# jzebedee/deltaq

Hardware: AMD Instinct MI355X
Metric: MB of text suffix-sorted per second (bit-exact SA) (higher is better)
Workload: dtype u8 text / u64 keys / int32 SA; 1 GPU; 256 MiB uniform-random bytes per GPU (splitmix64 seed 0x5EED0003+rank), int32 SA; bytes_per_gpu=268435456, residency=text and SA resident in HBM, rounds_after_initial_sort=1

## Files before the change

deltaq_amd/csrc/dq_bucket_sort.h:

```cpp
#pragma once
#include "dq_onesweep.h"
#include "dq_round0_plan.h"

namespace dq {

constexpr int kBktBins = kBktCap;
constexpr int kBktMaxBin = 48;

struct BucketFlags {
    unsigned long long overflow;
};

static __global__ __launch_bounds__(kBlock) void bucket_bounds_kernel(const uint64_t *__restrict__ W, int64_t n, int bshift,
                                                               int64_t C, int64_t X, int64_t ntiles,
                                                               int64_t *__restrict__ bounds,
                                                               BucketFlags *__restrict__ flags)
{
    const int64_t t = (int64_t)blockIdx.x * kBlock + threadIdx.x;
    if (t > ntiles) return;
    if (t == ntiles) { bounds[t] = n; return; }
    if (t == 0) { bounds[0] = 0; return; }
    const int64_t p = t * C;
    const uint64_t b = W[p - 1] >> bshift;
    int64_t lo = p, hi = p + X < n ? p + X : n;
// ... 17 lines not shown
    const int64_t b = (int64_t)blockIdx.x * kBlock + threadIdx.x;
    if (b > nbuckets) return;
    if (b == nbuckets) { bounds[ntiles] = n; return; }
    int64_t lo = 0, hi = n;
    while (lo < hi) {
        const int64_t mid = lo + ((hi - lo) >> 1);
        if ((int64_t)(W[mid] >> bshift) < b) lo = mid + 1; else hi = mid;
    }
    if (lo + X < n && (int64_t)(W[lo + X] >> bshift) == b) atomicOr(&flags->overflow, 2ull);
    if (b % g == 0) bounds[b / g] = lo;
}

template <int kThreads, int kItems, int kWavesPerSimd>
struct BktGeometry {
    static constexpr int threads = kThreads, items = kItems, waves = kWavesPerSimd;
    static constexpr int cap = kThreads * kItems;
    static constexpr int nb = 2 * cap;
    static_assert(cap < (1 << 16) && (nb / 2) % kThreads == 0 && kThreads % kWave == 0, "16-bit starts; whole bin words per thread");
};
using BktCoarse = BktGeometry<1024, kBktCap / 1024, 4>;
using BktFine = BktGeometry<512, kBktCapFine / 512, 4>;
static_assert(BktCoarse::cap == kBktCap && BktFine::cap == kBktCapFine, "the tiles are cut for these capacities");
constexpr int kBktArrBits = 6;
constexpr int kBktWalk = 4;
static_assert(kBktMaxBin < (1 << kBktArrBits), "arrival numbers must fit");

#ifdef DQ_BKT_PHASE_TIMING
__device__ long long *g_bkt_ts = nullptr;
#define DQ_BKT_PHASE(i) do { if (threadIdx.x == 0 && g_bkt_ts) g_bkt_ts[(long long)tile * 16 + (i)] = clock64(); } while (0)
#else
#define DQ_BKT_PHASE(i) do { } while (0)
#endif

template <typename IdxT, bool kExt = false, typename G = BktCoarse>
__global__ __launch_bounds__(G::threads, G::waves) void bucket_sort_kernel(
    const uint64_t *__restrict__ W, int ib, int lowbits, const int64_t *__restrict__ bounds, int64_t ntiles,
    IdxT *__restrict__ SA, uint32_t *__restrict__ ebits, BucketFlags *__restrict__ flags,
    const uint8_t *__restrict__ E = nullptr)
{
    constexpr int kCap = G::cap, kThreads = G::threads, kNB = G::nb, kItems = G::items;
    constexpr int kBinsPerThread = kNB / kThreads;
    constexpr int kWords = kBinsPerThread / 2;
    __shared__ uint32_t buf[kCap + kBktWalk];
    __shared__ uint32_t bins[kNB / 2 + 2];
    __shared__ uint32_t sufs[kCap];
    __shared__ uint32_t wtot[kThreads / kWave];
    __shared__ uint64_t s_edge[2];
    __shared__ uint32_t s_overflow;

    const uint32_t tid = threadIdx.x;
    const int lane = lane_id();
    const uint32_t wv = tid >> 6;
    const int bshift = ib + lowbits;
    const uint32_t imask = (uint32_t)((1ull << ib) - 1);
    const uint16_t *start16 = reinterpret_cast<const uint16_t *>(bins);

    int64_t tile = blockIdx.x;
    if (tile >= ntiles) return;
    int64_t lo_n = bounds[tile];
    uint32_t M_n = (uint32_t)(bounds[tile + 1] - lo_n);
    if (M_n > (uint32_t)kCap) M_n = 0;
    int64_t lo_nn = 0, hi_nn = 0;
    if (tile + gridDim.x < ntiles) { lo_nn = bounds[tile + gridDim.x]; hi_nn = bounds[tile + gridDim.x + 1]; }
    uint64_t wd[kItems];
#define DQ_BKT_FETCH()                                                            \
    do {                                                                          \
        const uint64_t *Wn = W + (M_n ? lo_n : 0);    \
        const uint32_t last_ = M_n > 0 ? M_n - 1 : 0;                             \
        _Pragma("unroll") for (int k = 0; k < kItems; ++k) {                   \
            const uint32_t e_ = (uint32_t)(k * kThreads) + tid;                \
            wd[k] = Wn[e_ < last_ ? e_ : last_];                                  \
        }                                                                         \
    } while (0)
#define DQ_BKT_REQUEST_NEXT()                                                     \
    do {                                                                          \
        lo_n = lo_nn;                                                             \
        M_n = (uint32_t)(hi_nn - lo_nn);                                          \
        if (M_n > (uint32_t)kCap) M_n = 0;                                     \
        DQ_BKT_FETCH();                                                           \
        if (tn + gridDim.x < ntiles) { lo_nn = bounds[tn + gridDim.x]; hi_nn = bounds[tn + gridDim.x + 1]; } \
    } while (0)
    DQ_BKT_FETCH();

    for (;;) {
        const int64_t lo = lo_n;
        const uint32_t M = M_n;
        const int64_t tn = tile + gridDim.x;
        if (M == 0) {
            if (tn >= ntiles) break;
            DQ_BKT_REQUEST_NEXT();
            tile = tn;
            continue;
        }
        DQ_BKT_PHASE(0);
        uint32_t ex[kExt ? kItems : 1];
        if (kExt) {
            const uint8_t *En = E + lo;
            const uint32_t last_ = M - 1;
#pragma unroll
            for (int k = 0; k < kItems; ++k) {
                const uint32_t e_ = (uint32_t)(k * kThreads) + tid;
                ex[k] = En[e_ < last_ ? e_ : last_];
            }
        }
        const int lowbits_t = kExt ? lowbits + 8 : lowbits;
        if (tid == 0) { s_edge[0] = wd[0]; s_overflow = 0; }
        if (tid == kThreads - 1) s_edge[1] = wd[kItems - 1];
        for (uint32_t i = tid; i < (uint32_t)(kNB / 2 + 2); i += kThreads) bins[i] = 0;
        __syncthreads();
        DQ_BKT_PHASE(1);
        const uint64_t kfirst = s_edge[0] >> bshift, klast = s_edge[1] >> bshift;
        const uint64_t range = (klast - kfirst + 1) << lowbits_t;
        const bool bad = range > (1ull << (32 - kBktArrBits));
        const uint32_t mult = bad ? 0u
            : (uint32_t)fminf((float)kNB * 4294967296.0f * __frcp_rn((float)range) * (1.0f - 0x1p-20f), 4294967040.0f);
        const uint64_t kbase = kfirst << lowbits;
        uint32_t key[kItems];
#pragma unroll
// ... 67 lines not shown
                        const uint32_t bin = __umulhi(key[k] >> kBktArrBits, mult);
                        const uint32_t s0 = start16[bin], s1 = start16[bin + 1];
                        r = s0;
                        if (s1 > s0 + 1) {
#pragma unroll
                        for (int q = 0; q < kBktWalk; ++q) {
                            const uint32_t o = buf[s0 + q];
                            const uint32_t less = (s0 + q < s1) & (o < key[k]);
                            r += less;
                            tie |= less & ((o >> kBktArrBits) == (key[k] >> kBktArrBits));
                        }
                        }
                        if (s1 > s0 + kBktWalk) {
#pragma clang loop vectorize(disable) interleave(disable) unroll(disable)
                            for (uint32_t j = s0 + kBktWalk; j < s1; ++j) {
                                const uint32_t o = buf[j];
                                const uint32_t less = o < key[k];
                                r += less;
                                tie |= less & ((o >> kBktArrBits) == (key[k] >> kBktArrBits));
                            }
                        }
                    }
                    fin[k] = e < M ? (r | (tie << 31)) : 0xffffffffu;
                }
                __syncthreads();
                DQ_BKT_PHASE(5);
#pragma unroll
                for (int k = 0; k < kItems; ++k) {
                    if (fin[k] != 0xffffffffu)
                        buf[fin[k] & 0x7fffffffu] = sufs[k * kThreads + tid] | (fin[k] & 0x80000000u);
                }
                __syncthreads();
                DQ_BKT_PHASE(6);
                IdxT *out = SA + lo;
                uint32_t v[kItems];
#pragma unroll
                for (int k = 0; k < kItems; ++k) {
                    const uint32_t e = (uint32_t)(k * kThreads) + tid;
                    v[k] = buf[e < M ? e : 0];
                }
                uint32_t ties = 0;
#pragma unroll
                for (int k = 0; k < kItems; ++k) {
                    const uint32_t e = (uint32_t)(k * kThreads) + tid;
                    if (e < M) out[e] = (IdxT)(v[k] & 0x7fffffffu);
                    ties |= (e < M && (v[k] >> 31)) ? (1u << k) : 0u;
                }
                while (ties) {
                    const int k = __builtin_ctz(ties);
                    ties &= ties - 1;
                    const uint64_t o = (uint64_t)(lo + k * kThreads + tid);
                    atomicOr(&ebits[o >> 5], 1u << ((uint32_t)o & 31u));
                }
                DQ_BKT_PHASE(7);
            }
        }
        if (tn >= ntiles) break;
        tile = tn;
        __syncthreads();
    }
#undef DQ_BKT_REQUEST_NEXT
#undef DQ_BKT_FETCH
}

}
```

deltaq_amd/csrc/dq_flags.h:

```cpp
#pragma once

#include <algorithm>
#include <cstdint>
#include <cstdlib>
#include <cstring>
#include <optional>
#include <string>

namespace dq {

struct Flags {
    bool debug = false;
    std::optional<int> trace;
    std::optional<int> hip_device;
    std::optional<int> numa_bind;
    std::optional<std::string> fault;
    std::optional<int> small_n;
    std::optional<int> no_many;
    std::optional<int> mid_many_min;
    std::optional<int> no_large_many;
    std::optional<int> large_many_min;
    std::optional<int> no_diff_many;
    std::optional<int> no_diff_mid_many;
    std::optional<int> diff_mid_many_min;
    std::optional<int> no_diff_large;
    std::optional<int> diff_large_min;
    std::optional<int> diff_large_table;
    std::optional<int> no_index_many;
    std::optional<int> index_many_min;
    std::optional<int> index_many_threads;
    std::optional<int> no_index_large;
    std::optional<int> index_large_min;
    std::optional<int> no_check_many;
    std::optional<int> no_bwt_many;
    std::optional<int> no_mtf_many;
    std::optional<int> no_huff_many;
    std::optional<int> mtf_short_max;
    bool no_list_buffers = false;
    bool text_copy = false;
    bool assume_doubled = false;
    bool no_twins = false;
    bool no_period_hint = false;
    std::optional<int> xcd_group;
    std::optional<int> packed;
    std::optional<int> key_bytes;
    std::optional<int> coded;
    std::optional<int> split;
    bool no_bucket = false;
    std::optional<int> bucket;
    std::optional<int> bucket_keybits;
    std::optional<int> bucket_ext;
    std::optional<int> bucket_tile;
    bool old_first_pass = false;
    bool no_fused_ties = false;
    std::optional<int> sparse;
    std::optional<int> binned_isa;
    bool no_binned_isa = false;
    std::optional<int> runs;
    bool no_small = false;
    bool no_wide_small = false;
    bool no_first_small = false;
    std::optional<int> mid_groups;
    bool no_l_shift = false;
    bool no_upd_words = false;
    std::optional<int> upd_bin;
    std::optional<int> upd_bin_min;
    std::optional<int> upd_window;
    std::optional<int> chain_steps;
    bool no_chain = false;
    bool force_rshift = false;
    std::optional<int> tail_max;
    std::optional<int> pair_chains;
    std::optional<int> pair_chains_min;
    std::optional<int> pair_maxg;
    std::optional<int> late_runs_min;
    bool no_late_runs = false;
    std::optional<int> run_period;
    bool search_wave = false;
    std::optional<int> search_ptab;
    bool no_wave_windows = false;
    bool no_poll = false;
    bool no_second_stage = false;
    std::optional<int> win_min;
    std::optional<int> win_second;
    std::optional<int> walk_on;
// ... 42 lines not shown
    f.large_many_min = num("DQ_LARGE_MANY_MIN", 1);
    f.no_diff_many = num("DQ_NO_DIFF_MANY", 0, 1);
    f.no_diff_mid_many = num("DQ_NO_DIFF_MID_MANY", 0, 1);
    f.diff_mid_many_min = num("DQ_DIFF_MID_MANY_MIN", 1);
    f.no_diff_large = num("DQ_NO_DIFF_LARGE", 0, 1);
    f.diff_large_min = num("DQ_DIFF_LARGE_MIN", 1);
    f.diff_large_table = num("DQ_DIFF_LARGE_TABLE", 0, 1);
    f.no_index_many = num("DQ_NO_INDEX_MANY", 0, 1);
    f.index_many_min = num("DQ_INDEX_MANY_MIN", 1);
    f.index_many_threads = num("DQ_INDEX_MANY_THREADS");
    f.no_index_large = num("DQ_NO_INDEX_LARGE", 0, 1);
    f.index_large_min = num("DQ_INDEX_LARGE_MIN", 1);
    f.no_check_many = num("DQ_NO_CHECK_MANY", 0, 1);
    f.no_bwt_many = num("DQ_NO_BWT_MANY", 0, 1);
    f.no_mtf_many = num("DQ_NO_MTF_MANY", 0, 1);
    f.no_huff_many = num("DQ_NO_HUFF_MANY", 0, 1);
    f.mtf_short_max = num("DQ_MTF_SHORT_MAX", 0);
    f.no_list_buffers = on("DQ_NO_LIST_BUFFERS");
    f.text_copy = on("DQ_TEXT_COPY");
    f.assume_doubled = on("DQ_ASSUME_DOUBLED");
    f.no_twins = on("DQ_NO_TWINS");
    f.no_period_hint = on("DQ_NO_PERIOD_HINT");

    f.xcd_group = num("DQ_XCD_GROUP", 0, 64);
    f.packed = num("DQ_PACKED");
    f.key_bytes = num("DQ_KEY_BYTES", 1, 8);
    f.coded = num("DQ_CODED");
    f.split = num("DQ_SPLIT");
    f.no_bucket = on("DQ_NO_BUCKET");
    f.bucket = num("DQ_BUCKET");
    f.bucket_keybits = num("DQ_BUCKET_KEYBITS");
    f.bucket_ext = num("DQ_BUCKET_EXT");
    f.bucket_tile = num("DQ_BUCKET_TILE", 0, 1);
    f.old_first_pass = on("DQ_OLD_FIRST_PASS");
    f.no_fused_ties = on("DQ_NO_FUSED_TIES");
    f.sparse = num("DQ_SPARSE");
    f.binned_isa = num("DQ_BINNED_ISA");
    f.no_binned_isa = on("DQ_NO_BINNED_ISA");
    f.runs = num("DQ_RUNS");

    f.no_small = on("DQ_NO_SMALL");
    f.no_wide_small = on("DQ_NO_WIDE_SMALL");
    f.no_first_small = on("DQ_NO_FIRST_SMALL");
    f.mid_groups = num("DQ_MID_GROUPS");
    f.no_l_shift = on("DQ_NO_L_SHIFT");
    f.no_upd_words = on("DQ_NO_UPD_WORDS");
    f.upd_bin = num("DQ_UPD_BIN", 0, 2);
    f.upd_bin_min = num("DQ_UPD_BIN_MIN", 1);
    f.upd_window = num("DQ_UPD_WINDOW");
    f.chain_steps = num("DQ_CHAIN_STEPS");
    f.no_chain = on("DQ_NO_CHAIN");
    f.force_rshift = on("DQ_FORCE_RSHIFT");

    f.tail_max = num("DQ_TAIL_MAX", 0);
    f.pair_chains = num("DQ_PAIR_CHAINS");
    f.pair_chains_min = num("DQ_PAIR_CHAINS_MIN", 1);
    f.pair_maxg = num("DQ_PAIR_MAXG", 2);
    f.late_runs_min = num("DQ_LATE_RUNS_MIN", 1);
    f.no_late_runs = on("DQ_NO_LATE_RUNS");
    f.run_period = num("DQ_RUN_PERIOD", 1);

    f.search_wave = on("DQ_SEARCH_WAVE");
    f.search_ptab = num("DQ_SEARCH_PTAB");
    f.no_wave_windows = on("DQ_NO_WAVE_WINDOWS");
    f.no_poll = on("DQ_NO_POLL");
    f.no_second_stage = on("DQ_NO_SECOND_STAGE");
// ... 78 lines not shown
```

deltaq_amd/csrc/dq_round0.h:

```cpp
#pragma once
#include "dq_sort_passes.h"
#include "dq_alpha_code.h"
#include "dq_ties.h"
#include "dq_bucket_sort.h"
#include "dq_xcd_rank.h"

namespace dq {
namespace {

constexpr int64_t kSgShortList = 1 << 20;
inline int mid_group_cap(int64_t list_len)
{
    if (const std::optional<int> g = flags().mid_groups) {
        return *g >= 1024 ? 1024 : *g >= 512 ? 512 : *g >= 256 ? 256 : 0;
    }
    return list_len >= kSgShortList ? 512 : 1024;
}
inline bool small_round_usable(int64_t n, int64_t mm, bool third_list_buffer)
{
    const Flags &F = flags();
    return !F.no_small && n < (1ll << 32) && (mm * 2 <= n || (third_list_buffer && !F.no_wide_small));
}

template <typename Fn>
int with_bool(bool on, Fn fn)
{
    return on ? fn(std::true_type{}) : fn(std::false_type{});
}

constexpr int kXcdHistAt = kRadixSize + 16;

template <typename IdxT>
struct Round0Out {
    uint64_t *Kr[2] = {nullptr, nullptr};
    IdxT *Vr[2] = {nullptr, nullptr};
    int64_t m = 0, h = 0;
    int rbits = 0;
    bool dense_built = false;
// ... 181 lines not shown
        DQ_TRY(isa_from_suffix_words<IdxT>(L, c, w, n, ib, k.kb, P0, keys));
        if (list_rank && o.m == 0) return DQ_OK;
        if (list_rank && small_round_usable(n, o.m, third) && rank32_direct) {
            o.first_rank32 = list_rank;
            return DQ_OK;
        }
        if (list_rank && small_round_usable(n, o.m, third)) {
            LAUNCH(L, DQ_K_KEY2_FROM_PAIRS, o.m, o.m * 12,
                   hipLaunchKernelGGL(widen_ranks_kernel, dim3(grid_for(o.m)), dim3(kBlock), 0, st,
                                      (const uint32_t *)list_rank, o.m, keys));
            return DQ_OK;
        }
        const bool with_key2 = !o.runs.runs_wanted;
        const int kbits = bit_length((uint64_t)(n - 1) + (uint64_t)k.kb);
        unsigned long long *cnt = reinterpret_cast<unsigned long long *>(w.totals + 3);
        HIP_TRY(hipMemsetAsync(cnt, 0, 8, st));
        const int64_t per = (int64_t)kPairThreads * kPairItems;
        LAUNCH(L, DQ_K_KEY2_FROM_PAIRS, n, n * 8 + o.m * (wb + 8 + wb),
               hipLaunchKernelGGL(key2_from_pairs_kernel<IdxT>, dim3((unsigned)((n + per - 1) / per)), dim3(kPairThreads),
                                  0, st, (const uint64_t *)P0, n, ib, (const IdxT *)w.ISA, (int64_t)k.kb, kbits, with_key2,
                                  keys, w.Va, cnt));
        o.keys_ready = with_key2;
        o.list_ungrouped = true;
        return DQ_OK;
    }

    int bucketed(bool *done)
    {
        *done = false;
        const Flags &F = flags();
        const BucketPlan b = plan_bucketed(s, F, k, coded, (int)wb);
        if (!b.applies) return DQ_OK;
        const int kb = k.kb, keybits = b.keybits, lowbits = b.lowbits;
        uint8_t *E[2] = {reinterpret_cast<uint8_t *>(w.Va), reinterpret_cast<uint8_t *>(w.Va) + align_up((size_t)n)};
        uint32_t *ebits = reinterpret_cast<uint32_t *>(w.Vb);
        TieCounters *ctr = reinterpret_cast<TieCounters *>(w.totals + 6);
        BucketFlags *bflags = reinterpret_cast<BucketFlags *>(&ctr->overflow);
        hipLaunchKernelGGL(text_digit_offsets_kernel, dim3(b.bbytes), dim3(kBlock), 0, st,
                           (const int64_t *)w.bytehist, (const uint8_t *)w.text, n, b.bbytes, w.digit_offset,
                           b.xcd_pass ? (const int64_t *)(w.bytehist + kXcdHistAt) : nullptr, b.xcd_pass ? w.xcd_offset : nullptr);
        HIP_TRY(hipGetLastError());
        if (c.ncu <= 0) {
            int v = 0;
            c.ncu = hipDeviceGetAttribute(&v, hipDeviceAttributeMultiprocessorCount, c.dev) == hipSuccess && v > 0 ? v : 256;
        }
        if (b.xcd_pass) {
            if (F.trace) fprintf(stderr, "[dq] XCD-local first pass (n=%lld, eighths of %lld)\n", (long long)n, (long long)xcd_eighth(n));
            if (sizeof(XcdRankCtl) > w.ctl_status_stride) return fail(DQ_ERR_HIP, "status buffer too small");
            LAUNCH(L, DQ_K_RADIX_RANK, n, n * (1 + 8),
                   hipLaunchKernelGGL(xcd_text_rank_kernel, dim3((unsigned)std::min<int64_t>(c.ncu, (n + kXcdTileN - 1) / kXcdTileN)),
                                      dim3(kXcdRankThreads), 0, st, reinterpret_cast<const uint32_t *>(w.text), K[1], n,
                                      ib + lowbits, keybits, ib, (const int64_t *)w.xcd_offset,
                                      reinterpret_cast<XcdRankCtl *>(w.ctl_status)));
        } else {
            DQ_TRY(b.ext ? rank_pass_ext<IdxT, kTextPackedExt>(L, w, text64(), (const uint8_t *)nullptr, K[1], E[1], n, 0, ib, ib + lowbits, keybits)
                       : rank_pass<IdxT, kTextPacked>(L, w, text64(), (const IdxT *)nullptr, K[1], (IdxT *)nullptr, n, 0, kb, ib,
                                                      nullptr, nullptr, ib + lowbits, keybits));
        }
        for (int p = 1; p < b.bbytes; ++p) {
            DQ_TRY(b.ext ? rank_pass_ext<IdxT, kKeysExt>(L, w, K[p & 1], E[p & 1], K[(p & 1) ^ 1], E[(p & 1) ^ 1], n, p, ib, ib + lowbits + 8 * p, keybits)
                       : rank_pass<IdxT, kKeys>(L, w, K[p & 1], (const IdxT *)nullptr, K[(p & 1) ^ 1], (IdxT *)nullptr, n, p, kb, ib,
                                                nullptr, nullptr, ib + lowbits + 8 * p, keybits));
        }
        uint64_t *Ks = K[b.bbytes & 1], *Kfree = K[(b.bbytes & 1) ^ 1];
        const uint8_t *Es = b.ext ? E[b.bbytes & 1] : nullptr;
        const FinishTiles ft = plan_finish_tiles(b, n, F);
        if (F.trace)
            fprintf(stderr, "[dq] bucket finish: %s geometry, %lld tiles of up to %lld words cut every %lld %s (n=%lld)\n", ft.fine ? "fine" : "coarse",
                    (long long)ft.ntiles, (long long)ft.cap, (long long)(ft.by_id ? ft.g : ft.Cf), ft.by_id ? "buckets" : "words", (long long)n);
        if ((size_t)ft.ntiles + 1 > finish_bounds_entries(n)) return fail(DQ_ERR_HIP, "tile bounds buffer too small");
        if (ft.by_id) {
            const int64_t nbuckets = (int64_t)1 << (8 * b.bbytes);
            LAUNCH(L, DQ_K_BUCKET_SORT, ft.ntiles, ft.ntiles * 16 * 8,
                   hipLaunchKernelGGL(bucket_bounds_by_id_kernel, dim3((unsigned)((nbuckets + 1 + kBlock - 1) / kBlock)), dim3(kBlock), 0,
                                      st, (const uint64_t *)Ks, n, ib + lowbits, ft.g, b.X, nbuckets, ft.ntiles, w.bkt_bounds, bflags));
        } else {
            LAUNCH(L, DQ_K_BUCKET_SORT, ft.ntiles, ft.ntiles * 16 * 8,
                   hipLaunchKernelGGL(bucket_bounds_kernel, dim3((unsigned)((ft.ntiles + 1 + kBlock - 1) / kBlock)), dim3(kBlock), 0,
                                      st, (const uint64_t *)Ks, n, ib + lowbits, ft.Cf, b.X, ft.ntiles, w.bkt_bounds, bflags));
        }
        auto finish = [&](auto kExt, auto geometry) -> int {
            using G = decltype(geometry);
            auto kernel = bucket_sort_kernel<IdxT, decltype(kExt)::value, G>;
            const int groups = resident_groups(&c.bkt_groups[ft.fine][b.ext][sizeof(IdxT) == 8], (const void *)kernel, G::threads, c.dev);
            LAUNCH(L, DQ_K_BUCKET_SORT, n, n * ((b.ext ? 9 : 8) + wb) + n / 8,
                   hipLaunchKernelGGL(kernel, dim3((unsigned)std::min<int64_t>(ft.ntiles, groups)), dim3(G::threads), 0, st,
                                      (const uint64_t *)Ks, ib, lowbits, (const int64_t *)w.bkt_bounds, ft.ntiles, d_sa, ebits, bflags, Es));
            return DQ_OK;
        };
        if (ft.fine) {
            DQ_TRY(finish(std::false_type{}, BktFine{}));
        } else {
            DQ_TRY(with_bool(b.ext, [&](auto kExt) -> int { return finish(kExt, BktCoarse{}); }));
        }
        if (b.ext && F.trace) fprintf(stderr, "[dq] bucketed round 0 with %d + 8 key bits per suffix (n=%lld)\n", keybits, (long long)n);
        bool overflow = false;
        DQ_TRY(collect_ties(ebits, nullptr, Kfree, &overflow, Ks, false, b.hb));
        if (overflow) {
            if (F.trace) fprintf(stderr, "[dq] bucketed round 0 gave up (n=%lld): plain digit passes\n", (long long)n);
            DQ_TRY(prepare_status<IdxT>(L, w, n, kMaxPasses));
            HIP_TRY(hipMemsetAsync(w.Vb, 0, (size_t)(tie_words() + 1) * 8, st));
            HIP_TRY(hipMemsetAsync(w.totals, 0, 64, st));
            o.m = 0; o.fin_cap = 0; o.fin_left = 0;
            return digit_tables(kb, false);
        }
        o.fin_done = o.m <= o.fin_cap;
        o.Kr[0] = Kfree; o.Kr[1] = Ks;
        o.h = b.hb;
        o.shallow_ties = true;
        *done = true;
        return DQ_OK;
    }

    int split(bool *done)
    {
        *done = false;
        if constexpr (sizeof(IdxT) != 4) {
            return DQ_OK;
        } else {
            if (!w.sp_top || !w.X || !w.RL) return DQ_OK;
            const int64_t cap = std::min<int64_t>(kFinCap, (n + 2) / (kSplitBuckets / 2));
            if (cap < 2) return DQ_OK;
            const uint32_t *t32 = reinterpret_cast<const uint32_t *>(w.text);
// ... 179 lines not shown
```

deltaq_amd/csrc/dq_round0_plan.h:

```cpp
#pragma once
#include <algorithm>
#include <cmath>
#include <cstddef>
#include <cstdint>

#include "dq_flags.h"

namespace dq {

constexpr int kKgramSamples = 1024;
constexpr int kBktCap = 12288;
constexpr int kBktCapFine = 6144;
constexpr int kSplitTop = 512;
constexpr int kSplitSub = 512;
constexpr int kSplitBuckets = kSplitTop * kSplitSub;
constexpr int kFinCap = 2048;
constexpr int64_t kSplitMinN = 5ll << 20;
constexpr int64_t kCodedMinN = 8ll << 20;
constexpr double kCodedMaxAvgLen = 5.8;
constexpr int kTieSamples = 4096;
constexpr int64_t kRound0MinN = 1 << 16;

inline int index_bits(int64_t n) { return n <= 1 ? 1 : 64 - __builtin_clzll((uint64_t)(n - 1)); }

// ... 96 lines not shown
            bbytes = 3;
            est *= pm;
            need = est + 6.0 * std::sqrt(est) + 64.0;
        }
        if (need > 5120 || (bbytes == 2 && !forced)) {
            if (!forced) return p;
            need = 5120;
        }
    }
    p.applies = true;
    p.keybits = keybits;
    p.bbytes = bbytes;
    p.X = std::min<int64_t>(((int64_t)need + 255) / 256 * 256, 5120);
    p.C = kBktCap - p.X;
    p.lowbits = keybits - 8 * bbytes;
    p.ntiles = (n + p.C - 1) / p.C;
    const bool room = (size_t)2 * (((size_t)n + 255) / 256 * 256) <= (size_t)(n + 2) * (size_t)idx_bytes;
    p.ext = keybits + 8 <= 56 && p.lowbits + 8 <= 18 && tied > 0.02 && room;
    if (F.bucket_ext) p.ext = *F.bucket_ext != 0 && keybits + 8 <= 56 && room;
    p.xcd_pass = !p.ext && !F.old_first_pass;
    p.hb = (keybits + (p.ext ? 8 : 0)) / 8;
    return p;
}

constexpr int64_t kBktFineMinN = 12ll << 20;
struct FinishTiles {
    bool fine = false;
    bool by_id = false;
    int64_t cap = 0;
    int64_t Cf = 0, g = 0;
    int64_t ntiles = 0;
};

inline FinishTiles plan_finish_tiles(const BucketPlan &b, int64_t n, const Flags &F)
{
    FinishTiles t;
    if (!b.applies) return t;
    const bool can = b.bbytes == 2 && !b.ext;
    t.fine = can && (F.bucket_tile ? *F.bucket_tile != 0 : !F.bucket.has_value() && n >= kBktFineMinN);
    t.cap = t.fine ? kBktCapFine : kBktCap;
    const int64_t Cf = t.cap - b.X;
    if (Cf >= b.X) {
        t.Cf = Cf;
        t.ntiles = (n + Cf - 1) / Cf;
    } else {
        t.by_id = true;
        t.g = std::min<int64_t>(t.cap / b.X, 64);
        const int64_t nbuckets = (int64_t)1 << (8 * b.bbytes);
        t.ntiles = (nbuckets + t.g - 1) / t.g;
    }
    return t;
}

inline size_t finish_bounds_entries(int64_t n)
{
    const size_t by_words = (size_t)n / (kBktCapFine / 2) + 4;
    return n < kRound0MinN ? by_words : std::max<size_t>(by_words, 65536 + 4);
}

inline bool fused_ties_wanted(int64_t n, KeyPlan k, const Flags &F)
{
    return k.packed && k.kb >= 2 && n >= kRound0MinN && !F.no_fused_ties && !F.sparse;
}

enum class DenseGuess { kNeither, kGuessDense, kTakeSample };

inline DenseGuess dense_guess(int64_t n, KeyPlan k)
{
    if (n < kRound0MinN || k.packed || k.kb != 8) return DenseGuess::kNeither;
    return n < (8 << 20) ? DenseGuess::kGuessDense : DenseGuess::kTakeSample;
}

inline bool predict_dense(DenseGuess g, int64_t tied_pairs, const Flags &F)
{
    if (F.sparse) return *F.sparse == 0;
    return g == DenseGuess::kGuessDense || (g == DenseGuess::kTakeSample && tied_pairs * 12 > kTieSamples);
}

inline bool binned_isa_pays(int64_t n, const Flags &F)
{
    const bool pays = F.binned_isa ? *F.binned_isa != 0 : n > (32ll << 20);
    return pays && n >= kRound0MinN && 2 * index_bits(n) <= 63 && !F.no_binned_isa;
}

// ... 20 lines not shown
```

deltaq_amd/csrc/dq_runtime.h:

```cpp
#pragma once
#include <hip/hip_runtime.h>

#include <algorithm>
#include <atomic>
#include <cctype>
#include <cmath>
#include <condition_variable>
#include <cstdio>
#include <cstdlib>
#include <cstring>
#include <chrono>
#include <mutex>
#include <string>
#include <memory>
#include <thread>
#include <vector>

#include <sched.h>

#include "../../include/dq_sufsort.h"
#include "dq_call_info.h"
#include "dq_flags.h"
#include "dq_work_lists.h"

// ... 33 lines not shown
    do {                                                                                \
        if (t_fault.hip_at && fault_hip())                                              \
            return fail(DQ_ERR_HIP, "injected fault (DQ_FAULT=hip) instead of " #expr); \
        hipError_t e_ = (expr);                                                         \
        if (e_ != hipSuccess)                                                           \
            return fail(e_ == hipErrorOutOfMemory ? DQ_ERR_OOM : DQ_ERR_HIP, #expr, e_); \
    } while (0)

#define DQ_TRY(...)                           \
    do {                                      \
        const int rc_ = (__VA_ARGS__);        \
        if (rc_ != DQ_OK) return rc_;         \
    } while (0)

struct KernelStat { int64_t launches = 0; double ms = 0; int64_t elems = 0; int64_t bytes = 0; };
inline std::mutex g_prof_mu;
inline KernelStat g_prof[DQ_K_COUNT];
inline std::atomic<int> g_prof_on{0};

inline const char *const kKernelNames[DQ_K_COUNT] = {
    "text_hist_kernel", "radix_hist_kernel", "radix_rank_kernel", "seg_fused_kernel",
    "tie_seam_kernel", "tie_collect_kernel", "small_group_finish_kernel", "small_group_round_kernel",
    "isa_update_kernel", "isa_from_pairs_kernel", "key2_from_pairs_kernel", "gather_key2_kernel",
    "gather_text_key_kernel", "isa_from_sa_kernel", "small_sufsort_kernel", "bucket_sort_kernel",
    "match_search_kernel", "pair_chain_kernels", "mid_group_round_kernel", "runlen_kernels",
    "split_pass_kernel", "bucket_finish_kernel", "split_round0_aux_kernels", "small_many_kernel"};

struct ProfRec { int cat; hipEvent_t a, b; int64_t elems, bytes; };

struct DeviceCtx {
    std::mutex mu;
    int dev = -1;
    int ncu = 0;
    int bkt_groups[2][2][2] = {};
    int many_groups[kAllClasses] = {};
    int check_many_groups[kCheckClasses] = {};
    int bwt_many_groups = 0;
    int mtf_many_groups[2] = {0, 0};
    int huff_many_groups = 0;
    int anchor_many_groups = 0;
    int anchor_mid_many_groups = 0;
    int anchor_index_many_groups[2] = {0, 0};
    int anchor_index_large_groups = 0;
    int anchor_pair_large_groups[2] = {0, 0};
    hipStream_t stream = nullptr;
    char *ws = nullptr;
    size_t ws_bytes = 0;
    int64_t *pinned = nullptr;
    uint8_t *pinned_io = nullptr;
    hipEvent_t readback = nullptr;
    std::vector<ProfRec> pending;
    std::vector<hipEvent_t> pool;
    std::mutex batch_mu;
    uint8_t *bslot_text[3] = {nullptr, nullptr, nullptr};
    int32_t *bslot_sa[3] = {nullptr, nullptr, nullptr};
    size_t bslot_cap = 0;
    hipStream_t b_in = nullptr, b_sort = nullptr, b_out = nullptr;
    std::mutex diff_mu;
    char *diff_dev = nullptr;
    size_t diff_dev_bytes = 0;
    char *diff_idx = nullptr;
    size_t diff_idx_bytes = 0;
    char *diff_pinned = nullptr;
    int scan_groups_cap = -1;
    int scan_groups_cap_narrow = -1;
    int scan_skip = 0;
// ... 364 lines not shown
```

deltaq_amd/csrc/dq_sort_passes.h:

```cpp
#pragma once
#include "dq_runtime.h"
#include "dq_round0_plan.h"
#include "dq_onesweep.h"
#include "dq_radix.h"
#include "dq_sa_kernels.h"
#include "dq_seg_fused.h"
#include "dq_small_groups.h"
#include "dq_runs.h"
#include "dq_isa_pairs.h"
#include "dq_split_round0.h"

namespace dq {
namespace {

constexpr int kSgChain = 8;

inline unsigned grid_for(int64_t items)
{
    return (unsigned)std::min<int64_t>((items + kBlock - 1) / kBlock, 256 * 16);
}

constexpr int64_t kSmallTileMaxM = 1ll << 20;
inline bool small_tiles(int64_t m) { return m <= kSmallTileMaxM; }
inline size_t status_tiles(size_t m)
// ... 4 lines not shown

template <typename IdxT>
struct Workspace {
    uint8_t *text;
    uint64_t *K0, *K1;
    IdxT *Va, *Vb, *ISA, *SAbuf;
    uint64_t *X;
    IdxT *Xs;
    int64_t *bkt_bounds;
    int64_t *totals;
    SmallGroupCounters *sg_ctr;
    uint32_t *hist_partial;
    uint16_t *codetab;
    uint32_t *pc_tiles;
    uint32_t *RL;
    uint32_t *run_lead, *run_carry;
    uint8_t *run_link;
    int64_t *digit_offset;
    int64_t *bytehist;
    int64_t *xcd_offset;
    char *ctl_status;
    size_t ctl_status_bytes;
    size_t ctl_status_stride;
    char *seg_status;
    size_t seg_status_bytes;
    uint64_t *sp_top, *sp_sub;
    unsigned long long *sp_cnt_a, *sp_cursor_a, *sp_cursor_b;
    int64_t *sp_off, *sp_out_base, *sp_ovf_src, *sp_ovf_dst;
    uint64_t *sp_low;
    uint8_t *sp_pure;
    uint32_t *sp_tile_first;
    ScanPart *sp_part;
    SplitCtl *sp_ctl;
    size_t bytes;
};

template <typename IdxT>
Workspace<IdxT> carve(char *base, int64_t n, bool with_sa, bool lists)
{
    Workspace<IdxT> w{};
    size_t off = 0;
    auto take = [&](size_t b) { char *p = base ? base + off : nullptr; off += align_up(b); return p; };
    const size_t un = (size_t)n;
    w.text = (uint8_t *)take(un + 64);
    w.K0 = (uint64_t *)take((un + 2) * 8);
    w.K1 = (uint64_t *)take((un + 2) * 8);
    w.Va = (IdxT *)take((un + 2) * sizeof(IdxT));
    w.Vb = (IdxT *)take((un + 2) * sizeof(IdxT));
    w.ISA = (IdxT *)take(un * sizeof(IdxT));
    w.SAbuf = with_sa ? (IdxT *)take(un * sizeof(IdxT)) : nullptr;
    if (lists) {
        w.X = (uint64_t *)take((un + 2) * 8);
        w.Xs = (IdxT *)take((un + 2) * sizeof(IdxT));
    }
    w.bkt_bounds = (int64_t *)take(finish_bounds_entries(n) * 8);
    w.totals = (int64_t *)take(64);
    w.sg_ctr = (SmallGroupCounters *)take((kSgChain + 2) * sizeof(SmallGroupCounters));
    w.hist_partial = (uint32_t *)take((size_t)kHistBlocks * kMaxPasses * kRadixSize * 4);
    w.digit_offset = (int64_t *)take((size_t)kMaxPasses * kRadixSize * 8);
    w.codetab = (uint16_t *)take(512);
    w.pc_tiles = (uint32_t *)take((un / 2048 + 4) * 8);
    if (sizeof(IdxT) == 4) {
        const size_t nchunks = un / kRunChunk + 2;
        w.RL = (uint32_t *)take(un * 4);
        w.run_lead = (uint32_t *)take(nchunks * 4);
        w.run_carry = (uint32_t *)take(nchunks * 4);
        w.run_link = (uint8_t *)take(nchunks);
    }
    w.bytehist = (int64_t *)take((size_t)(kRadixSize + 16 + kXcds * kRadixSize) * 8);
    w.xcd_offset = (int64_t *)take((size_t)kXcds * kRadixSize * 8);
    w.ctl_status_bytes = (size_t)kMaxPasses * align_up(256 + status_tiles(un) * kRadixSize * (un >= (1ull << 30) ? 8 : 4));
    w.ctl_status = take(w.ctl_status_bytes);
    w.seg_status_bytes = 256 + 3 * (un / kSegFusedTile + 2) * 8;
    w.seg_status = take(w.seg_status_bytes);
    if (sizeof(IdxT) == 4 && n >= kSplitMinN) {
        w.sp_top = (uint64_t *)take((size_t)kSplitTop * 8);
        w.sp_sub = (uint64_t *)take((size_t)kSplitBuckets * 8);
        w.sp_cnt_a = (unsigned long long *)take((size_t)kSplitTop * 8);
        w.sp_cursor_a = (unsigned long long *)take((size_t)kSplitTop * 8);
        w.sp_cursor_b = (unsigned long long *)take((size_t)kSplitBuckets * 8);
// ... 215 lines not shown
```

Baseline: 86540 MB/s.

## Scatter second radix pass directly into fixed-size per-bucket slots

```diff
diff --git a/deltaq_amd/csrc/dq_bucket_sort.h b/deltaq_amd/csrc/dq_bucket_sort.h
--- a/deltaq_amd/csrc/dq_bucket_sort.h
+++ b/deltaq_amd/csrc/dq_bucket_sort.h
@@ -73,12 +73,14 @@
 #define DQ_BKT_PHASE(i) do { } while (0)
 #endif
 
-template <typename IdxT, bool kExt = false, typename G = BktCoarse>
+template <typename IdxT, bool kExt = false, typename G = BktCoarse, bool kSlots = false>
 __global__ __launch_bounds__(G::threads, G::waves) void bucket_sort_kernel(
     const uint64_t *__restrict__ W, int ib, int lowbits, const int64_t *__restrict__ bounds, int64_t ntiles,
     IdxT *__restrict__ SA, uint32_t *__restrict__ ebits, BucketFlags *__restrict__ flags,
-    const uint8_t *__restrict__ E = nullptr)
+    const uint8_t *__restrict__ E = nullptr, const uint32_t *__restrict__ slot_base = nullptr,
+    const uint32_t *__restrict__ slot_count = nullptr, const uint32_t *__restrict__ slot_out = nullptr)
 {
+    static_assert(!(kSlots && kExt), "the slot route has no extra key byte");
     constexpr int kCap = G::cap, kThreads = G::threads, kNB = G::nb, kItems = G::items;
     constexpr int kBinsPerThread = kNB / kThreads;
     constexpr int kWords = kBinsPerThread / 2;
@@ -98,11 +100,23 @@
 
     int64_t tile = blockIdx.x;
     if (tile >= ntiles) return;
-    int64_t lo_n = bounds[tile];
-    uint32_t M_n = (uint32_t)(bounds[tile + 1] - lo_n);
+#define DQ_BKT_BOUNDS(t_, lo_, hi_, out_)                                         \
+    do {                                                                          \
+        if constexpr (kSlots) {                                                   \
+            lo_ = (int64_t)slot_base[t_];                                         \
+            hi_ = lo_ + (int64_t)slot_count[t_];                                  \
+            out_ = (int64_t)slot_out[t_];                                         \
+        } else {                                                                  \
+            lo_ = bounds[t_];                                                     \
+            hi_ = bounds[(t_) + 1];                                               \
+        }                                                                         \
+    } while (0)
+    int64_t lo_n, hi_n, out_n = 0;
+    DQ_BKT_BOUNDS(tile, lo_n, hi_n, out_n);
+    uint32_t M_n = (uint32_t)(hi_n - lo_n);
     if (M_n > (uint32_t)kCap) M_n = 0;
-    int64_t lo_nn = 0, hi_nn = 0;
-    if (tile + gridDim.x < ntiles) { lo_nn = bounds[tile + gridDim.x]; hi_nn = bounds[tile + gridDim.x + 1]; }
+    int64_t lo_nn = 0, hi_nn = 0, out_nn = 0;
+    if (tile + gridDim.x < ntiles) DQ_BKT_BOUNDS(tile + gridDim.x, lo_nn, hi_nn, out_nn);
     uint64_t wd[kItems];
 #define DQ_BKT_FETCH()                                                            \
     do {                                                                          \
@@ -116,15 +130,17 @@
 #define DQ_BKT_REQUEST_NEXT()                                                     \
     do {                                                                          \
         lo_n = lo_nn;                                                             \
+        if constexpr (kSlots) out_n = out_nn;                                     \
         M_n = (uint32_t)(hi_nn - lo_nn);                                          \
         if (M_n > (uint32_t)kCap) M_n = 0;                                     \
         DQ_BKT_FETCH();                                                           \
-        if (tn + gridDim.x < ntiles) { lo_nn = bounds[tn + gridDim.x]; hi_nn = bounds[tn + gridDim.x + 1]; } \
+        if (tn + gridDim.x < ntiles) DQ_BKT_BOUNDS(tn + gridDim.x, lo_nn, hi_nn, out_nn); \
     } while (0)
     DQ_BKT_FETCH();
 
     for (;;) {
         const int64_t lo = lo_n;
+        const int64_t olo = kSlots ? out_n : lo_n;
         const uint32_t M = M_n;
         const int64_t tn = tile + gridDim.x;
         if (M == 0) {
@@ -258,7 +274,7 @@
                 }
                 __syncthreads();
                 DQ_BKT_PHASE(6);
-                IdxT *out = SA + lo;
+                IdxT *out = SA + olo;
                 uint32_t v[kItems];
 #pragma unroll
                 for (int k = 0; k < kItems; ++k) {
@@ -275,7 +291,7 @@
                 while (ties) {
                     const int k = __builtin_ctz(ties);
                     ties &= ties - 1;
-                    const uint64_t o = (uint64_t)(lo + k * kThreads + tid);
+                    const uint64_t o = (uint64_t)(olo + k * kThreads + tid);
                     atomicOr(&ebits[o >> 5], 1u << ((uint32_t)o & 31u));
                 }
                 DQ_BKT_PHASE(7);
@@ -285,6 +301,7 @@
         tile = tn;
         __syncthreads();
     }
+#undef DQ_BKT_BOUNDS
 #undef DQ_BKT_REQUEST_NEXT
 #undef DQ_BKT_FETCH
 }
diff --git a/deltaq_amd/csrc/dq_flags.h b/deltaq_amd/csrc/dq_flags.h
--- a/deltaq_amd/csrc/dq_flags.h
+++ b/deltaq_amd/csrc/dq_flags.h
@@ -51,6 +51,7 @@
     std::optional<int> bucket_keybits;
     std::optional<int> bucket_ext;
     std::optional<int> bucket_tile;
+    std::optional<int> bucket_slots;
     bool old_first_pass = false;
     bool no_fused_ties = false;
     std::optional<int> sparse;
@@ -159,6 +160,7 @@
     f.bucket_keybits = num("DQ_BUCKET_KEYBITS");
     f.bucket_ext = num("DQ_BUCKET_EXT");
     f.bucket_tile = num("DQ_BUCKET_TILE", 0, 1);
+    f.bucket_slots = num("DQ_BUCKET_SLOTS", 0, 1);
     f.old_first_pass = on("DQ_OLD_FIRST_PASS");
     f.no_fused_ties = on("DQ_NO_FUSED_TIES");
     f.sparse = num("DQ_SPARSE");
diff --git a/deltaq_amd/csrc/dq_round0.h b/deltaq_amd/csrc/dq_round0.h
--- a/deltaq_amd/csrc/dq_round0.h
+++ b/deltaq_amd/csrc/dq_round0.h
@@ -4,6 +4,7 @@
 #include "dq_ties.h"
 #include "dq_bucket_sort.h"
 #include "dq_xcd_rank.h"
+#include "dq_slot_rank.h"
 
 namespace dq {
 namespace {
@@ -251,6 +252,14 @@
         const BucketPlan b = plan_bucketed(s, F, k, coded, (int)wb);
         if (!b.applies) return DQ_OK;
         const int kb = k.kb, keybits = b.keybits, lowbits = b.lowbits;
+        const SlotPlan sp = bucket_slots_fit(s, b, (int)wb);
+        const FinishTiles ft = plan_finish_tiles(b, n, F, sp.fits);
+        static_assert(sizeof(SlotRankCtl) <= (size_t)kHistBlocks * kMaxPasses * kRadixSize * 4, "the cursors live in the histogram scratch");
+        const bool slots = bucket_slots_wanted(sp, ft, F) && (uint64_t)sp.words <= slot_span_words_of(w) &&
+                           (size_t)(2 * kSlotBuckets + 5) * 4 <= finish_bounds_entries(n) * 8;
+        uint32_t *slot_base = reinterpret_cast<uint32_t *>(w.bkt_bounds), *slot_out = slot_base + kSlotBuckets + 4;
+        SlotRankCtl *sctl = reinterpret_cast<SlotRankCtl *>(w.hist_partial);
+        const int first = slots ? 0 : 1;
         uint8_t *E[2] = {reinterpret_cast<uint8_t *>(w.Va), reinterpret_cast<uint8_t *>(w.Va) + align_up((size_t)n)};
         uint32_t *ebits = reinterpret_cast<uint32_t *>(w.Vb);
         TieCounters *ctr = reinterpret_cast<TieCounters *>(w.totals + 6);
@@ -259,6 +268,14 @@
                            (const int64_t *)w.bytehist, (const uint8_t *)w.text, n, b.bbytes, w.digit_offset,
                            b.xcd_pass ? (const int64_t *)(w.bytehist + kXcdHistAt) : nullptr, b.xcd_pass ? w.xcd_offset : nullptr);
         HIP_TRY(hipGetLastError());
+        if (slots) {
+            if (F.trace)
+                fprintf(stderr, "[dq] second pass into bucket slots: %d x %d slots of %lld words (n=%lld)\n", sp.first, sp.second,
+                        (long long)b.X, (long long)n);
+            HIP_TRY(hipMemsetAsync(sctl, 0, sizeof(SlotRankCtl), st));
+            hipLaunchKernelGGL(slot_plan_kernel, dim3(kRadixSize + 1), dim3(kBlock), 0, st, (const int64_t *)w.bytehist, b.X, slot_base);
+            HIP_TRY(hipGetLastError());
+        }
         if (c.ncu <= 0) {
             int v = 0;
             c.ncu = hipDeviceGetAttribute(&v, hipDeviceAttributeMultiprocessorCount, c.dev) == hipSuccess && v > 0 ? v : 256;
@@ -268,27 +285,42 @@
             if (sizeof(XcdRankCtl) > w.ctl_status_stride) return fail(DQ_ERR_HIP, "status buffer too small");
             LAUNCH(L, DQ_K_RADIX_RANK, n, n * (1 + 8),
                    hipLaunchKernelGGL(xcd_text_rank_kernel, dim3((unsigned)std::min<int64_t>(c.ncu, (n + kXcdTileN - 1) / kXcdTileN)),
-                                      dim3(kXcdRankThreads), 0, st, reinterpret_cast<const uint32_t *>(w.text), K[1], n,
+                                      dim3(kXcdRankThreads), 0, st, reinterpret_cast<const uint32_t *>(w.text), K[first], n,
                                       ib + lowbits, keybits, ib, (const int64_t *)w.xcd_offset,
                                       reinterpret_cast<XcdRankCtl *>(w.ctl_status)));
         } else {
             DQ_TRY(b.ext ? rank_pass_ext<IdxT, kTextPackedExt>(L, w, text64(), (const uint8_t *)nullptr, K[1], E[1], n, 0, ib, ib + lowbits, keybits)
-                       : rank_pass<IdxT, kTextPacked>(L, w, text64(), (const IdxT *)nullptr, K[1], (IdxT *)nullptr, n, 0, kb, ib,
+                       : rank_pass<IdxT, kTextPacked>(L, w, text64(), (const IdxT *)nullptr, K[first], (IdxT *)nullptr, n, 0, kb, ib,
                                                       nullptr, nullptr, ib + lowbits, keybits));
         }
-        for (int p = 1; p < b.bbytes; ++p) {
+        if (slots) {
+            const int groups = resident_groups(&c.slot_rank_groups, (const void *)slot_rank_kernel, kSlotRankThreads, c.dev);
+            LAUNCH(L, DQ_K_RADIX_RANK, n, n * 16,
+                   hipLaunchKernelGGL(slot_rank_kernel, dim3((unsigned)std::min<int64_t>(groups, (n + kSlotTileN - 1) / kSlotTileN)),
+                                      dim3(kSlotRankThreads), 0, st, (const uint64_t *)K[0], K[1], n, ib + lowbits + 8, ib + lowbits,
+                                      (const int64_t *)w.digit_offset, (const uint32_t *)slot_base, sctl, bflags));
+        }
+        for (int p = 1; p < b.bbytes && !slots; ++p) {
             DQ_TRY(b.ext ? rank_pass_ext<IdxT, kKeysExt>(L, w, K[p & 1], E[p & 1], K[(p & 1) ^ 1], E[(p & 1) ^ 1], n, p, ib, ib + lowbits + 8 * p, keybits)
                        : rank_pass<IdxT, kKeys>(L, w, K[p & 1], (const IdxT *)nullptr, K[(p & 1) ^ 1], (IdxT *)nullptr, n, p, kb, ib,
                                                 nullptr, nullptr, ib + lowbits + 8 * p, keybits));
         }
-        uint64_t *Ks = K[b.bbytes & 1], *Kfree = K[(b.bbytes & 1) ^ 1];
+        uint64_t *Ks = slots ? K[1] : K[b.bbytes & 1], *Kfree = slots ? K[0] : K[(b.bbytes & 1) ^ 1];
         const uint8_t *Es = b.ext ? E[b.bbytes & 1] : nullptr;
-        const FinishTiles ft = plan_finish_tiles(b, n, F);
         if (F.trace)
             fprintf(stderr, "[dq] bucket finish: %s geometry, %lld tiles of up to %lld words cut every %lld %s (n=%lld)\n", ft.fine ? "fine" : "coarse",
                     (long long)ft.ntiles, (long long)ft.cap, (long long)(ft.by_id ? ft.g : ft.Cf), ft.by_id ? "buckets" : "words", (long long)n);
         if ((size_t)ft.ntiles + 1 > finish_bounds_entries(n)) return fail(DQ_ERR_HIP, "tile bounds buffer too small");
-        if (ft.by_id) {
+        if (slots) {
+            LAUNCH(L, DQ_K_BUCKET_SORT, ft.ntiles, ft.ntiles * 16,
+                   hipLaunchKernelGGL(slot_out_kernel, dim3(1), dim3(kSlotOutThreads), 0, st, sctl->cursor, (uint32_t)b.X, slot_out, bflags));
+            auto kernel = bucket_sort_kernel<IdxT, false, BktFine, true>;
+            const int groups = resident_groups(&c.bkt_slot_groups[sizeof(IdxT) == 8], (const void *)kernel, BktFine::threads, c.dev);
+            LAUNCH(L, DQ_K_BUCKET_SORT, n, n * (8 + wb) + n / 8,
+                   hipLaunchKernelGGL(kernel, dim3((unsigned)std::min<int64_t>(ft.ntiles, groups)), dim3(BktFine::threads), 0, st,
+                                      (const uint64_t *)Ks, ib, lowbits, (const int64_t *)nullptr, ft.ntiles, d_sa, ebits, bflags,
+                                      (const uint8_t *)nullptr, (const uint32_t *)slot_base, (const uint32_t *)sctl->cursor, (const uint32_t *)slot_out));
+        } else if (ft.by_id) {
             const int64_t nbuckets = (int64_t)1 << (8 * b.bbytes);
             LAUNCH(L, DQ_K_BUCKET_SORT, ft.ntiles, ft.ntiles * 16 * 8,
                    hipLaunchKernelGGL(bucket_bounds_by_id_kernel, dim3((unsigned)((nbuckets + 1 + kBlock - 1) / kBlock)), dim3(kBlock), 0,
@@ -304,10 +336,12 @@
             const int groups = resident_groups(&c.bkt_groups[ft.fine][b.ext][sizeof(IdxT) == 8], (const void *)kernel, G::threads, c.dev);
             LAUNCH(L, DQ_K_BUCKET_SORT, n, n * ((b.ext ? 9 : 8) + wb) + n / 8,
                    hipLaunchKernelGGL(kernel, dim3((unsigned)std::min<int64_t>(ft.ntiles, groups)), dim3(G::threads), 0, st,
-                                      (const uint64_t *)Ks, ib, lowbits, (const int64_t *)w.bkt_bounds, ft.ntiles, d_sa, ebits, bflags, Es));
+                                      (const uint64_t *)Ks, ib, lowbits, (const int64_t *)w.bkt_bounds, ft.ntiles, d_sa, ebits, bflags, Es,
+                                      (const uint32_t *)nullptr, (const uint32_t *)nullptr, (const uint32_t *)nullptr));
             return DQ_OK;
         };
-        if (ft.fine) {
+        if (slots) {
+        } else if (ft.fine) {
             DQ_TRY(finish(std::false_type{}, BktFine{}));
         } else {
             DQ_TRY(with_bool(b.ext, [&](auto kExt) -> int { return finish(kExt, BktCoarse{}); }));
diff --git a/deltaq_amd/csrc/dq_round0_plan.h b/deltaq_amd/csrc/dq_round0_plan.h
--- a/deltaq_amd/csrc/dq_round0_plan.h
+++ b/deltaq_amd/csrc/dq_round0_plan.h
@@ -152,7 +152,7 @@
     int64_t ntiles = 0;
 };
 
-inline FinishTiles plan_finish_tiles(const BucketPlan &b, int64_t n, const Flags &F)
+inline FinishTiles plan_finish_tiles(const BucketPlan &b, int64_t n, const Flags &F, bool slots_fit = false)
 {
     FinishTiles t;
     if (!b.applies) return t;
@@ -160,7 +160,12 @@
     t.fine = can && (F.bucket_tile ? *F.bucket_tile != 0 : !F.bucket.has_value() && n >= kBktFineMinN);
     t.cap = t.fine ? kBktCapFine : kBktCap;
     const int64_t Cf = t.cap - b.X;
-    if (Cf >= b.X) {
+    const bool force_by_id = t.fine && slots_fit && F.bucket_slots && *F.bucket_slots == 1;
+    if (force_by_id) {
+        t.by_id = true;
+        t.g = 1;
+        t.ntiles = (int64_t)1 << (8 * b.bbytes);
+    } else if (Cf >= b.X) {
         t.Cf = Cf;
         t.ntiles = (n + Cf - 1) / Cf;
     } else {
@@ -170,6 +175,45 @@
         t.ntiles = (nbuckets + t.g - 1) / t.g;
     }
     return t;
+}
+
+inline int64_t slot_span_words(int64_t n, int idx_bytes) { return (n + 2) * (int64_t)(8 + idx_bytes) / 8; }
+
+struct SlotPlan {
+    bool fits = false;
+    int first = 0, second = 0;
+    int64_t words = 0;
+};
+
+inline SlotPlan bucket_slots_fit(const TextStats &s, const BucketPlan &b, int idx_bytes)
+{
+    SlotPlan p;
+    if (!b.applies || b.bbytes != 2 || b.ext) return p;
+    p.first = s.sigma;
+    p.second = s.sigma + (s.hist[0] == 0 ? 1 : 0);
+    p.words = (int64_t)p.first * p.second * b.X;
+    p.fits = p.words <= slot_span_words(s.n, idx_bytes) && p.words < ((int64_t)1 << 32);
+    return p;
+}
+
+inline void slot_bases(const int64_t *hist , int64_t X, uint32_t *base )
+{
+    int ra[257], rb[257];
+    ra[0] = rb[0] = 0;
+    for (int d = 0; d < 256; ++d) {
+        ra[d + 1] = ra[d] + (hist[d] > 0 ? 1 : 0);
+        rb[d + 1] = rb[d] + (hist[d] > 0 || d == 0 ? 1 : 0);
+    }
+    for (int A = 0; A < 256; ++A)
+        for (int B = 0; B < 256; ++B)
+            base[A * 256 + B] = (uint32_t)(X * ((int64_t)ra[A] * rb[256] + (hist[A] > 0 ? rb[B] : 0)));
+    base[65536] = (uint32_t)(X * ra[256] * rb[256]);
+}
+
+inline bool bucket_slots_wanted(const SlotPlan &p, const FinishTiles &t, const Flags &F)
+{
+    if (F.bucket_slots && *F.bucket_slots == 0) return false;
+    return p.fits && t.fine && t.by_id && t.g == 1;
 }
 
 inline size_t finish_bounds_entries(int64_t n)
diff --git a/deltaq_amd/csrc/dq_runtime.h b/deltaq_amd/csrc/dq_runtime.h
--- a/deltaq_amd/csrc/dq_runtime.h
+++ b/deltaq_amd/csrc/dq_runtime.h
@@ -89,6 +89,8 @@
     std::mutex mu;
     int dev = -1;
     int ncu = 0;
+    int slot_rank_groups = 0;
+    int bkt_slot_groups[2] = {};
     int bkt_groups[2][2][2] = {};
     int many_groups[kAllClasses] = {};
     int check_many_groups[kCheckClasses] = {};
diff --git a/deltaq_amd/csrc/dq_slot_rank.h b/deltaq_amd/csrc/dq_slot_rank.h
--- /dev/null
+++ b/deltaq_amd/csrc/dq_slot_rank.h
@@ -0,0 +1,248 @@
+#pragma once
+#include "dq_bucket_sort.h"
+#include "dq_xcd_rank.h"
+
+namespace dq {
+
+constexpr int kSlotBuckets = 1 << 16;
+
+struct SlotRankCtl {
+    uint32_t ticket[kXcds];
+    uint32_t pad[64 - kXcds];
+    uint32_t cursor[kSlotBuckets];
+};
+
+static __global__ __launch_bounds__(kBlock) void slot_plan_kernel(const int64_t *__restrict__ bytehist, int64_t X,
+                                                           uint32_t *__restrict__ slot_base )
+{
+    __shared__ int tmp[kWavesPerBlock];
+    __shared__ int s_rank, s_present;
+    const int d = threadIdx.x, A = blockIdx.x;
+    const int pa = bytehist[d] > 0 ? 1 : 0, pb = (pa || d == 0) ? 1 : 0;
+    int na, nb;
+    const int ra = block_excl_sum(pa, tmp, &na);
+    __syncthreads();
+    const int rb = block_excl_sum(pb, tmp, &nb);
+    if (A == kRadixSize) {
+        if (d == 0) slot_base[kSlotBuckets] = (uint32_t)(X * na * nb);
+        return;
+    }
+    if (d == A) { s_rank = ra; s_present = pa; }
+    __syncthreads();
+    slot_base[A * kRadixSize + d] = (uint32_t)(X * ((int64_t)s_rank * nb + (s_present ? rb : 0)));
+}
+
+constexpr int kSlotOutThreads = 1024;
+static __global__ __launch_bounds__(kSlotOutThreads) void slot_out_kernel(uint32_t *__restrict__ count , uint32_t X,
+                                                                   uint32_t *__restrict__ out ,
+                                                                   BucketFlags *__restrict__ flags)
+{
+    constexpr int kPer = kSlotBuckets / kSlotOutThreads, kVec = kPer / 4;
+    __shared__ uint32_t wtot[kSlotOutThreads / kWave];
+    const int tid = threadIdx.x, lane = lane_id(), wv = tid >> 6;
+    uint4 *cv = reinterpret_cast<uint4 *>(count) + tid * kVec;
+    uint4 c[kVec];
+#pragma unroll
+    for (int i = 0; i < kVec; ++i) c[i] = cv[i];
+    uint32_t sum = 0, mx = 0;
+#pragma unroll
+    for (int i = 0; i < kVec; ++i) {
+        mx = max(max(max(c[i].x, c[i].y), max(c[i].z, c[i].w)), mx);
+        c[i].x = min(c[i].x, X); c[i].y = min(c[i].y, X); c[i].z = min(c[i].z, X); c[i].w = min(c[i].w, X);
+        sum += c[i].x + c[i].y + c[i].z + c[i].w;
+    }
+    if (mx > X) {
+        atomicOr(&flags->overflow, 2ull);
+#pragma unroll
+        for (int i = 0; i < kVec; ++i) cv[i] = c[i];
+    }
+    const uint32_t incl = wave_incl_sum(sum);
+    if (lane == kWave - 1) wtot[wv] = incl;
+    __syncthreads();
+    uint32_t run = incl - sum;
+    for (int i = 0; i < wv; ++i) run += wtot[i];
+    uint4 *ov = reinterpret_cast<uint4 *>(out) + tid * kVec;
+#pragma unroll
+    for (int i = 0; i < kVec; ++i) {
+        uint4 o;
+        o.x = run; run += c[i].x;
+        o.y = run; run += c[i].y;
+        o.z = run; run += c[i].z;
+        o.w = run; run += c[i].w;
+        ov[i] = o;
+    }
+    if (tid == kSlotOutThreads - 1) out[kSlotBuckets] = run;
+}
+
+#ifdef DQ_SLOT_PHASE_TIMING
+__device__ long long *g_slot_ts = nullptr;
+__device__ unsigned int g_slot_ts_next = 0;
+#define DQ_SLOT_PHASE(i) do { if (threadIdx.x == 0 && g_slot_ts) g_slot_ts[(long long)ts_row * 8 + (i)] = clock64(); } while (0)
+#else
+#define DQ_SLOT_PHASE(i) do { } while (0)
+#endif
+
+constexpr int kSlotRankThreads = 1024;
+constexpr int kSlotRankItems = 12;
+constexpr int kSlotTileN = kSlotRankThreads * kSlotRankItems;
+
+static __global__ __launch_bounds__(kSlotRankThreads, 1) void slot_rank_kernel(
+    const uint64_t *__restrict__ kin , uint64_t *__restrict__ wout, int64_t n,
+    int shift , int bshift ,
+    const int64_t *__restrict__ region , const uint32_t *__restrict__ slot_base ,
+    SlotRankCtl *__restrict__ ctl, BucketFlags *__restrict__ flags)
+{
+    constexpr int kThreads = kSlotRankThreads, kItems = kSlotRankItems, kTileN = kSlotTileN;
+    constexpr int kPerXcd = kRadixSize / kXcds;
+    __shared__ __attribute__((aligned(16))) uint64_t exch[kTileN];
+    __shared__ uint32_t cnt[kRadixSize];
+    __shared__ uint32_t tile_base[kRadixSize];
+    __shared__ uint32_t gofs[kRadixSize];
+    __shared__ uint32_t glim[kRadixSize];
+    __shared__ uint32_t wtmp[kRadixSize / kWave];
+    __shared__ uint32_t r_lo[kRadixSize], r_hi[kRadixSize], r_tiles[kRadixSize];
+    __shared__ uint32_t xs[kXcds][kPerXcd + 1];
+    __shared__ uint32_t s_lo, s_cnt;
+
+    const int tid = threadIdx.x;
+    const int w = tid >> 6;
+    const int lane = lane_id();
+    const uint32_t xcd = hw_xcc_id();
+
+    if (tid < kRadixSize) {
+        const int64_t lo = region[tid], hi = tid + 1 < kRadixSize ? region[tid + 1] : n;
+        r_lo[tid] = (uint32_t)lo;
+        r_hi[tid] = (uint32_t)hi;
+        r_tiles[tid] = (uint32_t)((hi - lo + kTileN - 1) / kTileN);
+        cnt[tid] = 0;
+    }
+    __syncthreads();
+    if (tid < kXcds) {
+        uint32_t run = 0;
+        for (int j = 0; j < kPerXcd; ++j) { xs[tid][j] = run; run += r_tiles[tid + kXcds * j]; }
+        xs[tid][kPerXcd] = run;
+    }
+    __syncthreads();
+
+    int tried = 0;
+    int32_t pend_e = -1;
+    uint32_t pend_t = 0;
+    auto issue = [&]() {
+        pend_e = -1;
+        for (; tried < kXcds; ++tried) {
+            const int32_t e = (int32_t)((xcd + (uint32_t)tried) & (kXcds - 1));
+            if (xs[e][kPerXcd] > 0) { pend_e = e; pend_t = atomicAdd(&ctl->ticket[e], 1u); return; }
+        }
+    };
+    auto resolve = [&]() {
+        while (pend_e >= 0) {
+            if (pend_t < xs[pend_e][kPerXcd]) {
+                int j = 0;
+                while (xs[pend_e][j + 1] <= pend_t) ++j;
+                const int B = pend_e + kXcds * j;
+                const uint32_t lo = r_lo[B] + (pend_t - xs[pend_e][j]) * (uint32_t)kTileN;
+                const uint32_t left = r_hi[B] - lo;
+                s_lo = lo;
+                s_cnt = left < (uint32_t)kTileN ? left : (uint32_t)kTileN;
+                return;
+            }
+            ++tried;
+            issue();
+        }
+        s_cnt = 0;
+    };
+
+    if (tid == 0) { issue(); resolve(); issue(); }
+    __syncthreads();
+    uint32_t lo = s_lo, valid = s_cnt;
+
+    uint64_t nw[kItems];
+    auto load_words = [&](uint32_t at, uint32_t m) {
+        if (m == 0) return;
+        const uint64_t *src = kin + at;
+#pragma unroll
+        for (int k = 0; k < kItems; ++k) {
+            const uint32_t q = (uint32_t)(k * kThreads + tid);
+            nw[k] = src[q < m ? q : m - 1];
+        }
+    };
+    load_words(lo, valid);
+#ifdef DQ_SLOT_PHASE_TIMING
+    __shared__ uint32_t s_row;
+#endif
+
+    while (valid > 0) {
+#ifdef DQ_SLOT_PHASE_TIMING
+        if (tid == 0) s_row = g_slot_ts ? atomicAdd(&g_slot_ts_next, 1u) : 0u;
+#endif
+        uint64_t key[kItems];
+#pragma unroll
+        for (int k = 0; k < kItems; ++k) key[k] = nw[k];
+        const uint32_t B = digit_of(key[0], bshift);
+        uint32_t sbase = 0, room = 0;
+        if (tid < kRadixSize) {
+            const uint32_t b = (uint32_t)tid * kRadixSize + B;
+            sbase = slot_base[b];
+            room = slot_base[b + 1] - sbase;
+        }
+        if (tid == 0) { resolve(); issue(); }
+        __syncthreads();
+#ifdef DQ_SLOT_PHASE_TIMING
+        const uint32_t ts_row = s_row;
+#endif
+        DQ_SLOT_PHASE(0);
+        const uint32_t next_lo = s_lo, next_valid = s_cnt;
+        load_words(next_lo, next_valid);
+
+        uint32_t pos[kItems];
+#pragma unroll
+        for (int k = 0; k < kItems; ++k)
+            pos[k] = atomicAdd(&cnt[digit_of(key[k], shift)], (uint32_t)(k * kThreads + tid) < valid ? 1u : 0u);
+        __syncthreads();
+        DQ_SLOT_PHASE(1);
+
+        uint32_t tot = 0, incl = 0, abase = 0;
+        if (tid < kRadixSize) {
+            tot = cnt[tid];
+            cnt[tid] = 0;
+            if (tot && room) abase = atomicAdd(&ctl->cursor[(uint32_t)tid * kRadixSize + B], tot);
+            incl = wave_incl_sum(tot);
+            if (lane == kWave - 1) wtmp[w] = incl;
+        }
+        __syncthreads();
+        uint32_t excl_tile = 0;
+        if (tid < kRadixSize) {
+            uint32_t off = 0;
+#pragma unroll
+            for (int i = 0; i < kRadixSize / kWave; ++i) if (i < w) off += wtmp[i];
+            excl_tile = off + incl - tot;
+            tile_base[tid] = excl_tile;
+        }
+        __syncthreads();
+
+#pragma unroll
+        for (int k = 0; k < kItems; ++k)
+            if ((uint32_t)(k * kThreads + tid) < valid) exch[pos[k] + tile_base[digit_of(key[k], shift)]] = key[k];
+        if (tid < kRadixSize) {
+            gofs[tid] = sbase + abase - excl_tile;
+            glim[tid] = excl_tile + (abase < room ? room - abase : 0u);
+            if (tot && abase + tot > room) atomicOr(&flags->overflow, 2ull);
+        }
+        __syncthreads();
+        DQ_SLOT_PHASE(2);
+#pragma unroll
+        for (int k = 0; k < kItems; ++k) key[k] = exch[k * kThreads + tid];
+
+#pragma unroll
+        for (int k = 0; k < kItems; ++k) {
+            const uint32_t q = (uint32_t)(k * kThreads + tid);
+            const uint32_t d = digit_of(key[k], shift);
+            if (q < valid && q < glim[d]) wout[gofs[d] + q] = key[k];
+        }
+        DQ_SLOT_PHASE(3);
+        lo = next_lo;
+        valid = next_valid;
+    }
+}
+
+}
diff --git a/deltaq_amd/csrc/dq_sort_passes.h b/deltaq_amd/csrc/dq_sort_passes.h
--- a/deltaq_amd/csrc/dq_sort_passes.h
+++ b/deltaq_amd/csrc/dq_sort_passes.h
@@ -60,8 +60,12 @@
     uint32_t *sp_tile_first;
     ScanPart *sp_part;
     SplitCtl *sp_ctl;
+    size_t slot_span_words;
     size_t bytes;
 };
+
+template <typename IdxT>
+inline uint64_t slot_span_words_of(const Workspace<IdxT> &w) { return (uint64_t)w.slot_span_words; }
 
 template <typename IdxT>
 Workspace<IdxT> carve(char *base, int64_t n, bool with_sa, bool lists)
@@ -72,8 +76,11 @@
     const size_t un = (size_t)n;
     w.text = (uint8_t *)take(un + 64);
     w.K0 = (uint64_t *)take((un + 2) * 8);
+    const size_t k1_at = off;
     w.K1 = (uint64_t *)take((un + 2) * 8);
+    const bool adjacent = off == k1_at + align_up((un + 2) * 8);
     w.Va = (IdxT *)take((un + 2) * sizeof(IdxT));
+    w.slot_span_words = adjacent ? (off - k1_at) / 8 : 0;
     w.Vb = (IdxT *)take((un + 2) * sizeof(IdxT));
     w.ISA = (IdxT *)take(un * sizeof(IdxT));
     w.SAbuf = with_sa ? (IdxT *)take(un * sizeof(IdxT)) : nullptr;
```

After: 91460 MB/s (median of 6 runs). 5.7% higher.
